# cy-rae/fast-slam

Measured on AMD Instinct MI355X. Metric: particle-updates/s, higher is better.
Workload: dtype f64

## Files before the change

fast-slam_amd/csrc/fs2_api.hip:

```cpp
#include <hip/hip_runtime.h>

#include <sched.h>
#include <unistd.h>

#include <algorithm>
#include <atomic>
#include <chrono>
#include <condition_variable>
#include <functional>
#include <cmath>
#include <cstdarg>
#include <cstdio>
#include <cstdlib>
#include <cstring>
#include <mutex>
#include <new>
#include <string>
#include <thread>
#include <tuple>
#include <vector>

#include "../../include/fs2.h"
#include "fs2_comm.hpp"
#include "fs2_frontend.hpp"
// ... 270 lines not shown
static void gm_free(GrowMem &g) {
    GmStep st{"free", g.mapped};
    size_t off = g.mapped;
    for (auto it = g.chunks.rbegin(); it != g.chunks.rend(); ++it) {
        off -= it->second;
        hipMemUnmap(g.base + off, it->second);
        gm_drop(g, it->second, it->first);
    }
    g.chunks.clear();
    if (g.base) hipMemAddressFree(g.base, g.reserved);
    g = GrowMem{};
}

struct Pool {
    const char *name;
    size_t item_bytes;
    int64_t id_limit;
    char *data = nullptr;
    int64_t n = 0;
    GrowMem vm;
    uint8_t *mark = nullptr;
    GrowMem mark_vm;
    uint32_t *freel = nullptr;
    GrowMem freel_vm;
    int64_t nfree = 0, cursor = 0;
    uint8_t epoch = 0;
    int64_t *bcnt = nullptr;
    int64_t bcnt_cap = 0;
    int64_t *nfree_dev = nullptr;

    int64_t room() const { return nfree - cursor; }
    int64_t live() const { return n - room(); }
    bool in_place() const { return vm.base && data == vm.base; }
    hipError_t next_epoch(hipStream_t s) {
        if (epoch == 255) {
            const hipError_t e = hipMemsetAsync(mark, 0, (size_t)n, s);
            if (e != hipSuccess) return e;
            epoch = 0;
        }
        epoch += 1;
        return hipSuccess;
    }
    bool mapped() const { return vm.base || mark_vm.base || freel_vm.base; }
    void release() {
        if (vm.base) gm_free(vm); else hipFree(data);
        if (mark_vm.base) gm_free(mark_vm); else hipFree(mark);
        if (freel_vm.base) gm_free(freel_vm); else hipFree(freel);
        hipFree(bcnt);
        hipFree(nfree_dev);
    }
};

}

struct MtCtx {
    fs2_mt_state in;
    double sigma = 0.0;
    int64_t N = 0, P = 0, A = 0, amb_cap = 0, pos0 = 0, have = 0, total = 0;
    int h0 = 0;
    fs2_mt_state *after = nullptr, *after_u0 = nullptr;
    double *u0_out = nullptr;
};

struct fs2_handle {
    fs2_config cfg{};
    int64_t n_global = 0, n = 0, first = 0;
    hipStream_t stream = nullptr;
    int cur = 0;
    double *x[2] = {}, *y[2] = {}, *yaw[2] = {}, *w[2] = {};
    int32_t *cnt[2] = {};
    Pool pages{"page", kPageBytes, (int64_t)kIdMask};
    Pool records{"record", kRecBytes, (int64_t)kRecIdLimit};
    Desc *pt[2] = {};
    uint32_t *bbox[2] = {};
    XDesc *rdesc = nullptr;
    XDesc *udesc = nullptr;
    size_t udesc_cap = 0;
    unsigned long long *xt_key = nullptr;
    uint32_t *xt_ref = nullptr, *xt_uidx = nullptr, *xt_cmask = nullptr, *xt_cbase = nullptr;
    uint32_t *xt_eslot = nullptr, *xt_ulist = nullptr;
    int64_t xt_cap = 0, xt_ecap = 0;
    SumFrame frame{-127.0f, 1.0f, 1.0f};
    float ext_seen = 0.0f;
    float *slb = nullptr;
    float *slb_pass = nullptr;
    uint32_t *ext_dev = nullptr;
    size_t rdesc_cap = 0;
    int rows = 0;
    uint32_t *sent_mask = nullptr;
    uint64_t collections = 0;
    int64_t u_recv = 0;
    int32_t *rank_d = nullptr, *rank_e = nullptr;
    int64_t *iblk = nullptr;
    int cap = 0, max_cap = kMaxSlots;
    double *wpart = nullptr, *part_sq = nullptr, *part_best_w = nullptr, *part_pose = nullptr;
    unsigned long long *cpart = nullptr;
    int64_t *part_best_i = nullptr;
    unsigned long long *part_slots = nullptr;
    int32_t *part_maxcnt = nullptr;
    double *cbuf = nullptr, *bsum = nullptr;
    DevStats *stats_dev = nullptr;
    char *post_host = nullptr, *post = nullptr;
    unsigned long long *post_flag = nullptr, *post_flag_dev = nullptr;
    unsigned long long post_seq = 0;
    PackPlan *plan = nullptr;
    DevStats *pub_stats = nullptr, *pub_stats_dev = nullptr;
    unsigned long long *pub_flag = nullptr, *pub_flag_dev = nullptr;
    unsigned long long pub_seq = 0;
    bool stats_clean = false;
    double *noise_dev = nullptr, *noise_pin = nullptr, *u0_dev = nullptr, *u0_pin = nullptr;
    struct MtWork {
        uint32_t *raw[2] = {};
        int64_t raw_cap[2] = {};
        int cur = 0;
        hipStream_t side = nullptr;
        hipEvent_t ev_words = nullptr, ev_pre = nullptr;
        bool pre_valid = false;
        uint32_t pre_key[2][624];
        int32_t pre_spos[2];
        int64_t pre_pos0[2];
        int64_t pre_total = 0;
        int32_t *boff = nullptr;
        int64_t boff_cap = 0;
        MtMeta *meta = nullptr, *meta_pin = nullptr;
        MtAmb *amb = nullptr, *amb_pin = nullptr;
        int64_t amb_cap = 0;
        uint32_t *words_pin = nullptr;
        int64_t *pidx = nullptr, *pidx_pin = nullptr;
        double *pval = nullptr, *pval_pin = nullptr;
        int64_t patch_cap = 0, pval_cap = 0;
        double *tab = nullptr;
        int64_t jJ = 0;
        int jG = 0;
        uint64_t *jpoly = nullptr;
        uint32_t *jwin = nullptr;
        bool tab_ready = false;
        bool armed = false;
        hipStream_t dstream = nullptr;
        hipEvent_t ev_in = nullptr, ev_noise = nullptr;
        bool deferred = false;
        MtCtx dc;
    } mt;
    int32_t *assoc_dev = nullptr;
    int64_t assoc_cap = 0;
    int32_t last_m = 0;
    uint64_t scan = 0;
    struct Pending {
        bool on = false;
        unsigned long long seq = 0;
        bool prof = false;
        int passes = 0;
        int32_t m = 0;
        uint64_t fixed_bytes = 0;
    } pending;
    struct TailCtx {
        int32_t M = 0;
        int passes = 0;
        uint64_t fixed_bytes = 0;
        bool prof = false;
        int evset = 0;
        int32_t want_collect = 0;
        bool has_u0 = false;
        int par = 0;
    };
    struct {
        bool on = false;
// ... 801 lines not shown
    for (int p = 0; p < G; ++p) {
        const bool so = p != keep && at(R, p, 0) > 0, ro = p != R && at(p, keep, 0) > 0;
        soff[p + 1] = soff[p] + (so ? arena_align((size_t)xfer_bytes(at(R, p, 0), at(R, p, 1), at(R, p, 2), at(R, p, 3))) : 0);
        roff[p + 1] = roff[p] + (ro ? arena_align((size_t)xfer_bytes(at(p, keep, 0), at(p, keep, 1), at(p, keep, 2),
                                                                      at(p, keep, 3))) : 0);
    }
    rc = ensure_arena(h, h->sarena, h->scap, soff[G]);
    if (!rc) rc = ensure_arena(h, h->rarena, h->rcap, roff[G]);
    if (rc) return rc;
    for (int p = 0; p < G; ++p) {
        rs.sbuf[p] = nullptr;
        T.ubase[p + 1] = T.ubase[p] + (p == keep ? 0 : at(R, p, 2));
        const int64_t K = at(R, p, 0), S = at(R, p, 1), U = at(R, p, 2), C = at(R, p, 3);
        if (log_xfer)
            std::fprintf(stderr,
                         "fs2 xfer scan %lld rank %d (shard %d -> %d) -> shard %d (rank %d)%s: %lld particles, "
                         "%lld rows, %lld pages, %lld covariances, %lld B\n",
                         (long long)h->scan, R, h->shard, keep, p, owner[p], p == keep ? " kept" : "", (long long)K,
                         (long long)S, (long long)U, (long long)C, (long long)(p == keep ? 0 : xfer_bytes(K, S, U, C)));
        if (p == keep || K == 0) continue;
        const size_t bytes = (size_t)xfer_bytes(K, S, U, C);
        rs.sbuf[p] = h->sarena + soff[p];
        sends.push_back({owner[p], rs.sbuf[p], bytes});
        nsend += K;
    }
    if (nsend > INT32_MAX) return set_err(&h->err, FS2_ERR_CAPACITY, "%lld particles to send", (long long)nsend);
    HIP_TRY(h, launch_pack_write(rs, s));
    rs.npeers = 0;
    int32_t kbase = 0;
    int64_t ubase = 0;
    for (int q = 0; q < G; ++q) {
        if (q == R) continue;
        const int64_t K = at(q, keep, 0), S = at(q, keep, 1), U = at(q, keep, 2), C = at(q, keep, 3);
        if (!K) continue;
        const size_t bytes = (size_t)xfer_bytes(K, S, U, C);
        char *rb = h->rarena + roff[q];
        recvs.push_back({q, rb, bytes});
        RecvPeer &pp = rs.peers[rs.npeers++];
        pp.hdr = reinterpret_cast<const PackHeader *>(rb);
        pp.idx = reinterpret_cast<const uint32_t *>(rb + xfer_idx_off(K));
        pp.pages = reinterpret_cast<const XferPage *>(rb + xfer_page_off(K, S));
        pp.covs = reinterpret_cast<const double2 *>(rb + xfer_cov_off(K, S, U));
        pp.K = (int32_t)K;
        pp.kbase = kbase;
        pp.U = U;
        pp.ubase = ubase;
        kbase += (int32_t)K;
        ubase += U;
    }
    rc = timed_exchange(h, sends, recvs, s);
    if (rc) return rc;
    h->n_recv = kbase;
    h->u_recv = ubase;
    if (h->profiling) {
        uint64_t np = 0, nr = 0, nu = 0, nb = 0;
        for (int p = 0; p < G; ++p) {
            if (p == keep) continue;
            np += at(R, p, 0);
            nr += at(R, p, 1);
            nu += at(R, p, 2);
            nb += at(R, p, 0) ? xfer_bytes(at(R, p, 0), at(R, p, 1), at(R, p, 2), at(R, p, 3)) : 0;
        }
        h->prof.migrations += np ? 1 : 0;
        h->prof.sent_particles += np;
        h->prof.sent_rows += nr;
        h->prof.sent_pages += nu;
        h->prof.sent_bytes += nb;
        h->prof.migrate_ms +=
            std::chrono::duration<double, std::milli>(std::chrono::steady_clock::now() - t_start).count();
    }
    rs.ao = shard_begin(h->n_global, G, keep);
    if (h->follow) {
        ResampleParams r2 = rs;
        r2.ranges_mode = 2;
        HIP_TRY(h, launch_resample_ranges(r2, s));
    }
    if (keep != h->shard) h->shard_moves += 1;
    h->shard = keep;
    h->first = rs.ao;
    for (int q = 0; q < G; ++q) h->rank_of[q] = (int8_t)owner[q];
    return FS2_OK;
}

static bool spatial_order(const double *lm, int L, std::vector<int32_t> &perm) {
    perm.resize(L);
    for (int j = 0; j < L; ++j) {
        perm[j] = j;
        if (!std::isfinite(lm[6 * j]) || !std::isfinite(lm[6 * j + 1])) return false;
    }
    struct Rec {
        static void go(const double *lm, int32_t *a, int n) {
            if (n <= kPageSlots) return;
            double x0 = INFINITY, x1 = -INFINITY, y0 = INFINITY, y1 = -INFINITY;
            for (int k = 0; k < n; ++k) {
                x0 = std::min(x0, lm[6 * a[k]]);
                x1 = std::max(x1, lm[6 * a[k]]);
                y0 = std::min(y0, lm[6 * a[k] + 1]);
                y1 = std::max(y1, lm[6 * a[k] + 1]);
            }
            const int ax = (x1 - x0 >= y1 - y0) ? 0 : 1;
            std::stable_sort(a, a + n, [&](int32_t u, int32_t v) { return lm[6 * u + ax] < lm[6 * v + ax]; });
            int h = ((n / 2 + kPageSlots - 1) / kPageSlots) * kPageSlots;
            if (h >= n) h = n - kPageSlots;
            go(lm, a, h);
            go(lm, a + h, n - h);
        }
    };
    Rec::go(lm, perm.data(), L);
    return true;
}

extern "C" {

int32_t fs2_abi_version(void) { return FS2_ABI_VERSION; }

#ifndef FS2_BUILD_ID
#define FS2_BUILD_ID "unknown"
#endif
const char *fs2_build_id(void) { return FS2_BUILD_ID; }

void fs2_config_default(fs2_config *c) {
    if (!c) return;
    std::memset(c, 0, sizeof *c);
    c->num_particles = 20;
    c->translation_noise = 0.0055;
    c->rotation_noise = 0.001;
    c->measurement_noise[0] = 0.001;
    c->measurement_noise[3] = 0.001;
    c->max_landmark_distance = 8.0;
    c->init_landmark_cov[0] = 0.1;
    c->init_landmark_cov[3] = 0.1;
    c->weight_floor = 1e-5;
    c->landmark_capacity = 64;
    c->max_landmark_capacity = 4096;
    c->device = 0;
    c->reduce_mode = FS2_REDUCE_AUTO;
    c->seed = 0x5EEDF5A2ull;
    c->record_assoc = 0;
    c->gate_filter = 1;
    c->rank = 0;
    c->world_size = 1;
}

const char *fs2_last_error(const fs2_handle *h) {
    if (h && !h->err.empty()) return h->err.c_str();
    return g_last_error.c_str();
}

static void free_handle(fs2_handle *h) {
    if (!h) return;
    int prev_dev = -1;
    if (hipGetDevice(&prev_dev) != hipSuccess) prev_dev = -1;
    if (prev_dev != h->cfg.device) (void)hipSetDevice(h->cfg.device);
    if (h->stream) hipStreamSynchronize(h->stream);
    if (h->mt.dstream) hipStreamSynchronize(h->mt.dstream);
    const bool vmm = h->pages.mapped() || h->records.mapped();
    if (vmm) hipDeviceSynchronize();
    if (h->refs_shared && h->tp && !h->tp->in_process()) {
        std::string e;
        if (h->tp->allgather(h->ep_dev, h->epochs_dev, 1, h->stream, &e) == FS2_OK) hipStreamSynchronize(h->stream);
        h->tp->unshare();
        if (h->tp->allgather(h->ep_dev, h->epochs_dev, 1, h->stream, &e) == FS2_OK) hipStreamSynchronize(h->stream);
    }
    for (int s = 0; s < 2; ++s) {
        hipFree(h->x[s]); hipFree(h->y[s]); hipFree(h->yaw[s]); hipFree(h->w[s]); hipFree(h->cnt[s]);
        hipFree(h->pt[s]);
        hipFree(h->bbox[s]);
    }
    hipFree(h->rdesc); hipFree(h->udesc);
    hipFree(h->xt_key); hipFree(h->xt_ref); hipFree(h->xt_uidx); hipFree(h->xt_cmask); hipFree(h->xt_cbase);
    hipFree(h->xt_eslot); hipFree(h->xt_ulist);
    hipFree(h->sent_mask);
    h->pages.release();
    h->records.release();
    if (vmm) hipDeviceSynchronize();
    hipFree(h->slb); hipFree(h->slb_pass); hipFree(h->ext_dev);
    hipFree(h->rank_d); hipFree(h->rank_e); hipFree(h->iblk);
    hipFree(h->mlo); hipFree(h->mhi); hipFree(h->out_src); hipFree(h->runs); hipFree(h->runs_n);
    hipFree(h->rec); hipFree(h->recs); hipFree(h->totals); hipFree(h->xrow); hipFree(h->xmat);
    hipFree(h->sarena);
    hipFree(h->rarena);
    hipFree(h->cand); hipFree(h->ncand);
    hipFree(h->uinfo); hipFree(h->uol); hipFree(h->seql); hipFree(h->udelta); hipFree(h->ugl);
    hipFree(h->bD); hipFree(h->bC); hipFree(h->bM); hipFree(h->bpd); hipFree(h->bpc);
    hipFree(h->uel); hipFree(h->bE); hipFree(h->bpe);
    hipFree(h->sout); hipFree(h->np_leaf); hipFree(h->part_w); hipFree(h->np_part); hipFree(h->np_tail);
    hipFree(h->urec); hipFree(h->sentry);
    hipFree(h->dch_send); hipFree(h->dch_recv); hipFree(h->recx); hipFree(h->recxs); hipFree(h->est_base);
    hipFree(h->uop); hipFree(h->np_tail_g);
    hipFree(h->peers_dev); hipFree(h->ep_dev); hipFree(h->epochs_dev);
    hipFree(h->part_pose);
    hipFree(h->gen_dev); hipFree(h->sets_dev); hipFree(h->go_dev);
// ... 1017 lines not shown
                                        (long long)capacity, (long long)need);
    if (m_out) *m_out = h->last_m;
    HIP_TRY(h, hipStreamSynchronize(h->stream));
    if (need) HIP_TRY(h, hipMemcpy(idx, h->assoc_dev, sizeof(int32_t) * need, hipMemcpyDeviceToHost));
    return FS2_OK;
}

static hipMemcpyKind kind_in(int32_t where) {
    return where == FS2_DEVICE ? hipMemcpyDeviceToDevice : hipMemcpyHostToDevice;
}
static hipMemcpyKind kind_out(int32_t where) {
    return where == FS2_DEVICE ? hipMemcpyDeviceToDevice : hipMemcpyDeviceToHost;
}

int fs2_set_state(fs2_handle *h, int64_t first, int64_t count, const double *x, const double *y,
                  const double *yaw, const double *w, const int32_t *cnt, const double *lm,
                  int32_t lm_cap, int32_t where) {
    if (!h) return set_err(nullptr, FS2_ERR_ARG, "null handle");
    if (h->pending.on) return set_err(&h->err, FS2_ERR_STATE, "a submitted scan is pending (fs2_iterate_wait first)");
    if (first < 0 || count < 0 || first + count > h->n)
        return set_err(&h->err, FS2_ERR_ARG, "range [%lld, %lld) outside %lld local particles",
                       (long long)first, (long long)(first + count), (long long)h->n);
    if ((cnt == nullptr) != (lm == nullptr) || (lm && lm_cap < 0))
        return set_err(&h->err, FS2_ERR_ARG, "cnt and lm must be given together");
    HIP_TRY(h, hipSetDevice(h->cfg.device));
    {
        const int rcm = mt_finish(h);
        h->mt.armed = false;
        if (rcm) return rcm;
    }
    hipStream_t s = h->stream;
    const int c = h->cur;
    HIP_TRY(h, hipStreamSynchronize(s));
    if (count == 0) return FS2_OK;
    const size_t b8 = sizeof(double) * count;
    if (x) HIP_TRY(h, copy_sync(h, h->x[c] + first, x, b8, kind_in(where)));
    if (y) HIP_TRY(h, copy_sync(h, h->y[c] + first, y, b8, kind_in(where)));
    if (yaw) HIP_TRY(h, copy_sync(h, h->yaw[c] + first, yaw, b8, kind_in(where)));
    if (w) HIP_TRY(h, copy_sync(h, h->w[c] + first, w, b8, kind_in(where)));
    if (cnt) {
        std::vector<int32_t> hc(count);
        HIP_TRY(h, hipMemcpy(hc.data(), cnt, sizeof(int32_t) * count,
                             where == FS2_DEVICE ? hipMemcpyDeviceToHost : hipMemcpyHostToHost));
        int32_t mx = 0;
        for (int32_t v : hc) {
            if (v < 0 || v > lm_cap) return set_err(&h->err, FS2_ERR_ARG, "count %d outside [0, %d]", v, lm_cap);
            mx = std::max(mx, v);
        }
        int rc = grow_rows(h, mx);
        if (rc) return rc;
        const int32_t rows_each = std::max(1, (mx + kPageSlots - 1) / kPageSlots);
        h->cnt_upper = std::max(h->cnt_upper, mx);
        {
            int64_t used = 0;
            for (int32_t v : hc) used += v;
            h->appends_since_rcollect += used;
            if ((int64_t)h->imported.size() != h->n) h->imported.assign((size_t)h->n, 0);
            bool replaced = h->scan > 0;
            for (int64_t k = first; k < first + count; ++k) {
                replaced |= h->imported[(size_t)k] != 0;
                h->imported[(size_t)k] = 1;
            }
            if (replaced) h->rcollect_exact = false;
        }
        const int64_t per = (int64_t)std::max(1, lm_cap) * 6 * 8;
        const int64_t chunk = std::max<int64_t>(1, (256ll << 20) / per);
        double *stage = nullptr;
        int32_t *cstage = nullptr, *perm_dev = nullptr;
        HIP_TRY(h, hipMemsetAsync(h->ext_dev, 0, sizeof(uint32_t), s));
        HIP_TRY(h, hipMalloc(&stage, (size_t)std::min(chunk, count) * per));
        HIP_TRY(h, hipMalloc(&cstage, sizeof(int32_t) * std::min(chunk, count)));
        HIP_TRY(h, hipMalloc(&perm_dev, sizeof(int32_t) * std::max(1, lm_cap)));
        std::vector<double> rep((size_t)std::max(1, lm_cap) * 6);
        std::vector<int32_t> perm;
        int rc2 = FS2_OK;
        for (int64_t o = 0; o < count && rc2 == FS2_OK; o += chunk) {
            const int64_t k = std::min(chunk, count - o);
            hipError_t e = copy_sync(h, stage, lm + o * lm_cap * 6, (size_t)k * per, kind_in(where));
            if (e == hipSuccess) e = hipMemcpy(cstage, hc.data() + o, sizeof(int32_t) * k, hipMemcpyHostToDevice);
            int32_t perm_len = -1;
            if (e == hipSuccess && h->cfg.gate_filter && hc[o] > kPageSlots) {
                e = hipMemcpy(rep.data(), lm + o * lm_cap * 6, sizeof(double) * 6 * (size_t)hc[o],
                              where == FS2_DEVICE ? hipMemcpyDeviceToHost : hipMemcpyHostToHost);
                if (e == hipSuccess && spatial_order(rep.data(), hc[o], perm)) {
                    perm_len = hc[o];
                    e = hipMemcpy(perm_dev, perm.data(), sizeof(int32_t) * perm_len, hipMemcpyHostToDevice);
                }
            }
            PageAlloc pa{};
            rc2 = reserve_recs(h, k * std::max(1, lm_cap), &pa);
            if (rc2) break;
            rc2 = reserve_pages(h, k * rows_each, &pa);
            if (rc2) break;
            if (e == hipSuccess)
                e = launch_import(stage, cstage, first + o, k, lm_cap, h->map(), pa, rows_each, h->cnt[c], h->ext_dev,
                                  perm_len > 0 ? perm_dev : nullptr, perm_len, s);
            if (e == hipSuccess) e = hipStreamSynchronize(s);
            if (e != hipSuccess) rc2 = set_err(&h->err, FS2_ERR_HIP, "state import failed: %s", hipGetErrorString(e));
        }
        hipFree(stage);
        hipFree(cstage);
        hipFree(perm_dev);
        if (rc2) return rc2;
        uint32_t eb = 0;
        HIP_TRY(h, hipMemcpy(&eb, h->ext_dev, sizeof eb, hipMemcpyDeviceToHost));
        float ext = 0.0f;
        std::memcpy(&ext, &eb, sizeof ext);
        h->ext_seen = std::max(h->ext_seen, ext);
#ifdef FS2_AB_POW2_CELL
        float cell = 1.0f / 64.0f;
        while (127.0f * cell < 1.25f * h->ext_seen && cell < 65536.0f) cell *= 2.0f;
#else
        float cell = (float)std::max(1.0, std::ceil(1.25 * (double)h->ext_seen / 127.0 * 64.0)) / 64.0f;
        if (!(cell < 65536.0f)) cell = 65536.0f;
#endif
        if (cell != h->frame.cell) h->frame = SumFrame{-127.0f * cell, cell, 1.0f / cell};
        HIP_TRY(h, launch_bbox_build(h->map(), h->cnt[c], s));
    }
    HIP_TRY(h, hipStreamSynchronize(s));
    return FS2_OK;
}

int fs2_update_known_landmarks(fs2_handle *h, double eps, double min_fraction, double *centres, int64_t cap,
                               int64_t *n_clusters) {
    if (!h || !n_clusters || (cap > 0 && !centres) || !(eps > 0.0))
        return set_err(h ? &h->err : nullptr, FS2_ERR_ARG, "fs2_update_known_landmarks: bad arguments");
    if (h->pending.on) return set_err(&h->err, FS2_ERR_STATE, "a submitted scan is pending (fs2_iterate_wait first)");
    if (h->cfg.world_size > 1)
        return set_err(&h->err, FS2_ERR_STATE, "update_known_landmarks needs every particle on one rank");
    HIP_TRY(h, hipSetDevice(h->cfg.device));
    hipStream_t s = h->stream;
    HIP_TRY(h, hipStreamSynchronize(s));
    double2 *pts = nullptr;
    int64_t np = 0;
    HIP_TRY(h, gather_map_points(h->map(), h->cnt[h->cur], h->n, &pts, &np, s));
    const double avg = (double)np / (double)h->n_global;
    const double ms = avg * min_fraction;
    if (!(ms >= 1.0)) {
        (void)hipFree(pts);
        *n_clusters = -1;
        return FS2_OK;
    }
    int32_t status = 0;
    int64_t K = 0;
    double *dcent = nullptr;
    hipError_t e = hipMalloc(&dcent, sizeof(double) * 2 * std::max<int64_t>(cap, 1));
    if (e == hipSuccess)
        e = cluster_points(pts, np, eps, (int64_t)ms, dcent, cap, &K, nullptr, &status, s);
    if (e == hipSuccess && K <= cap && K > 0)
        e = hipMemcpy(centres, dcent, sizeof(double) * 2 * K, hipMemcpyDeviceToHost);
    (void)hipFree(pts);
    (void)hipFree(dcent);
    if (e != hipSuccess) return set_err(&h->err, FS2_ERR_HIP, "update_known_landmarks: %s", hipGetErrorString(e));
    if (status == 1) return set_err(&h->err, FS2_ERR_ARG, "Input contains NaN or infinity");
    if (status == 2) return set_err(&h->err, FS2_ERR_ARG, "landmark coordinates span too many eps-cells");
    *n_clusters = K;
    if (K > cap) return set_err(&h->err, FS2_ERR_ARG, "%lld clusters, centre buffer holds %lld", (long long)K,
                                (long long)cap);
    return FS2_OK;
}

int fs2_get_state(fs2_handle *h, int64_t first, int64_t count, double *x, double *y, double *yaw,
                  double *w, int32_t *cnt, double *lm, int32_t lm_cap, int32_t where) {
    if (!h) return set_err(nullptr, FS2_ERR_ARG, "null handle");
    if (h->pending.on) return set_err(&h->err, FS2_ERR_STATE, "a submitted scan is pending (fs2_iterate_wait first)");
    if (first < 0 || count < 0 || first + count > h->n)
        return set_err(&h->err, FS2_ERR_ARG, "range outside local particles");
    HIP_TRY(h, hipSetDevice(h->cfg.device));
// ... 995 lines not shown
        HIP_TRY(h, hipMemcpyAsync(mt.raw[nx], mt.raw[mt.cur] + kMtN * kb1, 4 * (size_t)keep,
                                  hipMemcpyDeviceToDevice, mt.side));
        {
            int64_t made = 0;
            const int rcf = mt_fill(h, mt.raw[nx], keep, want, mt.side, &made);
            if (rcf) return rcf;
            want = made;
        }
        HIP_TRY(h, hipEventRecord(mt.ev_pre, mt.side));
        std::memcpy(mt.pre_key[0], after->key, sizeof mt.pre_key[0]);
        std::memcpy(mt.pre_key[1], after_u0->key, sizeof mt.pre_key[1]);
        mt.pre_spos[0] = after->pos;
        mt.pre_spos[1] = after_u0->pos;
        mt.pre_pos0[0] = after->pos;
        mt.pre_pos0[1] = kMtN * (kb2 - kb1) + after_u0->pos;
        mt.pre_total = want;
        mt.pre_valid = true;
    }
    const uint32_t wu[2] = {meta.w_u0[0], meta.w_u0[1]};
    const double hi = 1.0 / (double)h->n_global;
    const double u0 = 0.0 + (hi - 0.0) * mt_double(mt_temper(wu[0]), mt_temper(wu[1]));
    *h->u0_pin = u0;
    HIP_TRY(h, hipMemcpyAsync(h->u0_dev, h->u0_pin, 8, hipMemcpyHostToDevice, s));
    if (c.u0_out) *c.u0_out = u0;
    return FS2_OK;
}

static int mt_finish(fs2_handle *h) {
    auto &mt = h->mt;
    if (!mt.deferred) return FS2_OK;
    mt.deferred = false;
    const int rc = mt_end(h, mt.dc, mt.dstream);
    HIP_TRY(h, hipEventRecord(mt.ev_noise, mt.dstream));
    HIP_TRY(h, hipStreamWaitEvent(h->stream, mt.ev_noise, 0));
    if (rc) return rc;
    mt.armed = true;
    return FS2_OK;
}

int fs2_mt_draw(fs2_handle *h, const fs2_mt_state *in, double sigma, fs2_mt_state *after,
                fs2_mt_state *after_u0, double *u0_out) {
    if (!h) return set_err(nullptr, FS2_ERR_ARG, "null handle");
    HIP_TRY(h, hipSetDevice(h->cfg.device));
    int rc = mt_finish(h);
    if (rc) return rc;
    h->mt.armed = false;
    MtCtx c;
    rc = mt_begin(h, in, sigma, after, after_u0, u0_out, h->stream, c);
    if (rc) return rc;
    rc = mt_end(h, c, h->stream);
    if (rc) return rc;
    h->mt.armed = true;
    return FS2_OK;
}

int fs2_mt_draw_deferred(fs2_handle *h, const fs2_mt_state *in, double sigma, fs2_mt_state *after,
                         fs2_mt_state *after_u0, double *u0_out) {
    if (!h) return set_err(nullptr, FS2_ERR_ARG, "null handle");
    HIP_TRY(h, hipSetDevice(h->cfg.device));
    auto &mt = h->mt;
    int rc = mt_finish(h);
    if (rc) return rc;
    mt.armed = false;
    if (!mt.dstream) {
        HIP_TRY(h, hipStreamCreateWithFlags(&mt.dstream, hipStreamNonBlocking));
        HIP_TRY(h, hipEventCreateWithFlags(&mt.ev_in, hipEventDisableTiming));
        HIP_TRY(h, hipEventCreateWithFlags(&mt.ev_noise, hipEventDisableTiming));
    }
    HIP_TRY(h, hipEventRecord(mt.ev_in, h->stream));
    HIP_TRY(h, hipStreamWaitEvent(mt.dstream, mt.ev_in, 0));
    MtCtx &c = mt.dc;
    rc = mt_begin(h, in, sigma, after, after_u0, u0_out, mt.dstream, c);
    if (rc) return rc;
    mt.deferred = true;
    return FS2_OK;
}

int fs2_debug_mt_jump(const uint32_t key[624], uint64_t J, uint32_t out[624]) {
    if (!key || !out) return set_err(nullptr, FS2_ERR_ARG, "fs2_debug_mt_jump: null argument");
    if (!mt_jump_host(key, J, out)) return set_err(nullptr, FS2_ERR_STATE, "MT19937 characteristic polynomial not found");
    return FS2_OK;
}

int64_t fs2_release_cached_memory(void) { return (int64_t)g_chunks.release(); }

int fs2_debug_vm_fail_after_relocate(int32_t on) {
    g_vm_fail_after_relocate.store(on ? 1 : 0);
    return FS2_OK;
}

int fs2_debug_refuse_peer_maps(fs2_handle *h) {
    if (!h) return set_err(nullptr, FS2_ERR_ARG, "null handle");
    if (h->refs_shared || h->refs_off)
        return set_err(&h->err, FS2_ERR_STATE, "fs2_debug_refuse_peer_maps: the pools are mapped already");
    h->refuse_maps = true;
    return FS2_OK;
}

int fs2_debug_noise(fs2_handle *h, double *out) {
    if (!h || !out) return set_err(h ? &h->err : nullptr, FS2_ERR_ARG, "fs2_debug_noise: null argument");
    HIP_TRY(h, hipSetDevice(h->cfg.device));
    {
        const int rcm = mt_finish(h);
        if (rcm) return rcm;
    }
    HIP_TRY(h, hipMemcpyAsync(h->noise_pin, h->noise_dev, sizeof(double) * h->n, hipMemcpyDeviceToHost, h->stream));
    HIP_TRY(h, hipStreamSynchronize(h->stream));
    std::memcpy(out, h->noise_pin, sizeof(double) * h->n);
    return FS2_OK;
}

int64_t fs2_debug_check_guards(fs2_handle *h, char *first_bad, int64_t len) {
    if (!h) return set_err(nullptr, FS2_ERR_ARG, "fs2_debug_check_guards: null handle");
    if (first_bad && len > 0) first_bad[0] = 0;
    HIP_TRY(h, hipSetDevice(h->cfg.device));
    HIP_TRY(h, hipStreamSynchronize(h->stream));
    std::vector<unsigned char> buf(kGuardBytes);
    int64_t bad = 0;
    for (const auto &g : h->guards) {
        HIP_TRY(h, hipMemcpy(buf.data(), g.at, kGuardBytes, hipMemcpyDeviceToHost));
        int64_t k = 0;
        for (unsigned char c : buf) k += c != (unsigned char)kGuardByte;
        if (k && first_bad && len > 0 && !first_bad[0]) std::snprintf(first_bad, (size_t)len, "%s", g.name);
        bad += k;
    }
    return bad;
}

int fs2_debug_weights(fs2_handle *h, int32_t other, double *out) {
    if (!h || !out) return set_err(h ? &h->err : nullptr, FS2_ERR_ARG, "fs2_debug_weights: null argument");
    HIP_TRY(h, hipSetDevice(h->cfg.device));
    HIP_TRY(h, hipStreamSynchronize(h->stream));
    HIP_TRY(h, hipMemcpy(out, h->w[other ? 1 - h->cur : h->cur], sizeof(double) * (size_t)h->n, hipMemcpyDeviceToHost));
    return FS2_OK;
}

int64_t fs2_debug_out_src(fs2_handle *h, int32_t *out, int64_t capacity) {
    if (!h || !out || capacity < h->n)
        return set_err(h ? &h->err : nullptr, FS2_ERR_ARG, "fs2_debug_out_src: null argument or capacity < n");
    HIP_TRY(h, hipSetDevice(h->cfg.device));
    HIP_TRY(h, hipStreamSynchronize(h->stream));
    HIP_TRY(h, hipMemcpy(out, h->out_src, sizeof(int32_t) * (size_t)h->n, hipMemcpyDeviceToHost));
    return h->n;
}

int fs2_debug_mt_log(int32_t device, const double *x, int64_t n, double *out, int32_t *amb, int32_t on_host) {
    if (n < 0 || (n > 0 && (!x || !out || !amb))) return set_err(nullptr, FS2_ERR_ARG, "fs2_debug_mt_log: bad arguments");
    if (on_host) {
        double thi[kMtLogTab], tlo[kMtLogTab];
        for (int k = 0; k < kMtLogTab; ++k) {
            const DD l = mt_log_tab_entry(k);
            thi[k] = l.hi;
            tlo[k] = l.lo;
        }
        for (int64_t k = 0; k < n; ++k) {
            bool a = false;
            out[k] = mt_log(x[k], thi, tlo, &a);
            amb[k] = a ? 1 : 0;
        }
        return FS2_OK;
    }
    if (n == 0) return FS2_OK;
    std::lock_guard<std::mutex> lk(g_scratch_mu);
    const size_t b8 = al16((size_t)n * 8);
    Scratch *sc = nullptr;
    int rc = scratch_get(device, 2 * b8 + al16((size_t)n * 4), &sc);
// ... 762 lines not shown
```

fast-slam_amd/fast_slam_2/_native.py:

```python
from __future__ import annotations

import ctypes as C
import os
import sys

import numpy as np

_PKG = os.path.dirname(os.path.abspath(__file__))
LIB_PATH = os.environ.get("FS2_LIB", os.path.join(os.path.dirname(_PKG), "lib", "libfs2.so"))

FS2_OK = 0
FS2_ERR_ARG = -1
FS2_ERR_HIP = -2
FS2_ERR_OOM = -3
FS2_ERR_LINALG = -4
FS2_ERR_STATE = -5
FS2_ERR_COMM = -6
FS2_ERR_CAPACITY = -7

FS2_REDUCE_AUTO = 0
FS2_REDUCE_SEQUENTIAL = 1
FS2_REDUCE_PARALLEL = 2
FS2_REDUCE_EXACT = 3
FS2_HOST = 0
# ... 146 lines not shown
    def __init__(self, code, msg):
        super().__init__(f"libfs2 error {code}: {msg}")
        self.code = code


_dp = C.POINTER(C.c_double)
_ip = C.POINTER(C.c_int32)
_vp = C.c_void_p
_H = C.c_void_p

SIGNATURES = [
    ("fs2_abi_version", C.c_int32, []),
    ("fs2_build_id", C.c_char_p, []),
    ("fs2_config_default", None, [C.POINTER(fs2_config)]),
    ("fs2_create", C.c_int, [C.POINTER(fs2_config), C.POINTER(_H)]),
    ("fs2_destroy", None, [_H]),
    ("fs2_last_error", C.c_char_p, [_H]),
    ("fs2_iterate", C.c_int, [_H, C.c_double, C.c_double, _vp, _vp, C.c_int32, _vp, _vp, _dp,
                              C.POINTER(fs2_iter_stats)]),
    ("fs2_iterate_submit", C.c_int, [_H, C.c_double, C.c_double, _vp, _vp, C.c_int32, _vp, _vp]),
    ("fs2_iterate_wait", C.c_int, [_H, _dp, C.POINTER(fs2_iter_stats)]),
    ("fs2_mt_draw", C.c_int, [_H, C.POINTER(fs2_mt_state), C.c_double, C.POINTER(fs2_mt_state),
                              C.POINTER(fs2_mt_state), _dp]),
    ("fs2_mt_draw_deferred", C.c_int, [_H, C.POINTER(fs2_mt_state), C.c_double, C.POINTER(fs2_mt_state),
                                       C.POINTER(fs2_mt_state), _dp]),
    ("fs2_get_state", C.c_int, [_H, C.c_int64, C.c_int64, _vp, _vp, _vp, _vp, _vp, _vp, C.c_int32,
                                C.c_int32]),
    ("fs2_set_state", C.c_int, [_H, C.c_int64, C.c_int64, _vp, _vp, _vp, _vp, _vp, _vp, C.c_int32,
                                C.c_int32]),
    ("fs2_snapshot_save", C.c_int, [_H, _vp, C.c_int64, C.POINTER(C.c_int64)]),
    ("fs2_snapshot_save_select", C.c_int, [_H, _vp, C.c_int64, _vp, C.c_int64, C.POINTER(C.c_int64)]),
    ("fs2_snapshot_load", C.c_int, [_H, _vp, C.c_int64]),
    ("fs2_snapshot_check", C.c_int, [_vp, C.c_int64, C.POINTER(fs2_snapshot_info)]),
    ("fs2_get_assoc", C.c_int, [_H, _ip, C.c_int64, _ip]),
    ("fs2_shard_info", C.c_int, [_H, C.POINTER(C.c_int64), C.POINTER(C.c_int64),
                                 C.POINTER(C.c_int32)]),
    ("fs2_synchronize", C.c_int, [_H]),
    ("fs2_set_profiling", C.c_int, [_H, C.c_int32]),
    ("fs2_get_profile", C.c_int, [_H, C.POINTER(fs2_profile)]),
    ("fs2_icp", C.c_int, [C.c_int32, _dp, C.c_int32, _dp, C.c_int32, C.c_int32, C.c_double, _dp,
                          _dp, _ip]),
    ("fs2_icp_submit", C.c_int, [C.c_int32, _dp, C.c_int32, _dp, C.c_int32, C.c_int32, C.c_double,
                                 C.POINTER(C.c_int64)]),
    ("fs2_icp_wait", C.c_int, [C.c_int32, C.c_int64, _dp, _dp, _ip]),
    ("fs2_icp_batched", C.c_int, [C.c_int32, C.c_int32, C.c_int32, _vp, _vp, C.c_int32,
                                  C.c_double, _vp, _vp, _vp, C.c_int32]),
    ("fs2_best_fit_transform", C.c_int, [C.c_int32, _dp, _dp, C.c_int32, _dp, _dp]),
    ("fs2_line_filter", C.c_int, [C.c_int32, _dp, C.c_int32, _dp, C.c_int32, _dp]),
    ("fs2_gaussian_taps", C.c_int32, [C.c_double, C.c_double, _dp, C.c_int32]),
    ("fs2_associate", C.c_int, [C.c_int32, _dp, _dp, C.c_int32, C.c_double, _ip]),
    ("fs2_mahalanobis", C.c_int, [C.c_int32, _dp, _dp, _dp, C.c_int32, _dp]),
    ("fs2_cluster_points", C.c_int, [C.c_int32, _vp, C.c_int64, C.c_double, C.c_int64, _vp, C.c_int64,
                                     C.POINTER(C.c_int64), _vp, C.c_int32]),
    ("fs2_update_known_landmarks", C.c_int, [_H, C.c_double, C.c_double, _dp, C.c_int64,
                                             C.POINTER(C.c_int64)]),
    ("fs2_frontend", C.c_int, [C.c_int32, C.c_int32, _vp, _vp, C.c_int32, _dp, C.c_int32, C.c_int32,
                               C.POINTER(fs2_frontend_out)]),
    ("fs2_repr_doubles", C.c_int, [C.c_int32, _vp, C.c_int64, _vp, _vp, C.c_int32]),
    ("fs2_poses_json", C.c_int, [C.c_int32, _vp, _vp, _vp, C.c_int64, C.c_int32, _vp, C.c_int64,
                                 C.POINTER(C.c_int64), C.c_int32]),
    ("fs2_particles_json", C.c_int, [_H, C.c_int64, C.c_int64, C.c_int32, _vp, C.c_int64,
                                     C.POINTER(C.c_int64)]),
    ("fs2_debug_json_times", C.c_int, [C.c_int32, _vp]),
    ("fs2_pose_moments", C.c_int, [_H, C.c_int32, _vp, _vp, _vp, _vp]),
    ("fs2_pose_density", C.c_int, [_H, C.c_int32, C.c_double, C.c_double, C.c_double, C.c_int32, C.c_int32, _vp,
                                   C.POINTER(C.c_int32), C.POINTER(C.c_uint64)]),
    ("fs2_density_scale", C.c_int, [C.c_double, C.c_int64, C.POINTER(C.c_int32)]),
    ("fs2_debug_posterior_times", C.c_int, [C.c_int32, _vp]),
    ("fs2_map_summary", C.c_int, [_H, _vp, _vp]),
    ("fs2_map_density", C.c_int, [_H, C.c_int32, C.c_double, C.c_double, C.c_double, C.c_int32, C.c_int32, _vp,
                                  C.POINTER(C.c_int32), C.POINTER(C.c_uint64)]),
    ("fs2_debug_map_times", C.c_int, [C.c_int32, _vp]),
    ("fs2_debug_philox", C.c_int, [C.c_int32, C.c_int64, _vp, _vp, _vp]),
    ("fs2_debug_normals", C.c_int, [C.c_int32, C.c_uint64, C.c_uint64, C.c_uint64, C.c_int64, _vp]),
    ("fs2_debug_mt_log", C.c_int, [C.c_int32, _vp, C.c_int64, _vp, _vp, C.c_int32]),
    ("fs2_debug_refuse_peer_maps", C.c_int, [_H]),
    ("fs2_debug_vm_fail_after_relocate", C.c_int, [C.c_int32]),
    ("fs2_release_cached_memory", C.c_int64, []),
    ("fs2_debug_noise", C.c_int, [_H, _vp]),
    ("fs2_debug_out_src", C.c_int64, [_H, _vp, C.c_int64]),
    ("fs2_debug_weights", C.c_int, [_H, C.c_int32, _vp]),
    ("fs2_debug_check_guards", C.c_int64, [_H, C.c_char_p, C.c_int64]),
    ("fs2_debug_mt_jump", C.c_int, [_vp, C.c_uint64, _vp]),
    ("fs2_comm_unique_id", C.c_int, [C.POINTER(C.c_uint8)]),
    ("fs2_plan_ranges", C.c_int, [_vp, C.c_int64, C.c_int64, C.c_int64, C.c_double, C.c_double, _vp, _vp]),
    ("fs2_plan_sends", C.c_int, [_vp, _vp, _vp, C.c_int64, C.c_int64, C.c_int32, C.c_int32, _vp, _vp, _vp]),
]

_lib = None


HIP_RUNTIME = None


def _wheel_hip_version(torch_dir):
    try:
        for line in open(os.path.join(torch_dir, "version.py")):
            if line.startswith("hip"):
                v = line.split("=", 1)[1].strip().strip("'\"")
                return None if v in ("None", "") else v
    except OSError:
        pass
    return None


def _system_hip_version():
    try:
        return open(os.path.join(os.environ.get("ROCM_PATH", "/opt/rocm"), ".info", "version")).read().strip()
    except OSError:
        return None


def _share_torch_hip_runtime():
    global HIP_RUNTIME
    want = os.environ.get("FS2_HIP_RUNTIME", "").strip().lower()
    sysv = _system_hip_version()
    HIP_RUNTIME = ("system", None, sysv)
    if want == "system":
        return
    torch_dirs = []
    if "torch" in sys.modules and getattr(sys.modules["torch"], "__file__", None):
        torch_dirs = [os.path.dirname(sys.modules["torch"].__file__)]
    else:
        try:
            import importlib.util
            spec = importlib.util.find_spec("torch")
        except Exception:
            spec = None
        if spec is not None and spec.submodule_search_locations:
            torch_dirs = list(spec.submodule_search_locations)
    for d in torch_dirs:
        p = os.path.join(d, "lib", "libamdhip64.so")
        if not os.path.exists(p):
            continue
        try:
            C.CDLL(p, mode=C.RTLD_GLOBAL)
        except OSError:
            return
        wv = _wheel_hip_version(d)
        HIP_RUNTIME = ("torch-wheel", p, wv)
        if wv and sysv and wv.split(".")[:2] != sysv.split(".")[:2]:
            import warnings
            warnings.warn(f"libfs2 runs on PyTorch's HIP runtime {wv} ({p}), not the system ROCm {sysv} it "
                          f"was compiled against (one runtime per process; FS2_HIP_RUNTIME=system opts out)",
                          RuntimeWarning, stacklevel=3)
        break
    if os.environ.get("FS2_VERBOSE"):
        print(f"[fs2] HIP runtime: {HIP_RUNTIME}", file=sys.stderr)


def load():
    global _lib
    if _lib is not None:
        return _lib
    if not os.path.exists(LIB_PATH):
        raise ImportError(f"libfs2.so not found at {LIB_PATH}; build it with "
                          f"`python fast-slam_amd/build.py` (there is no CPU fallback)")
    _share_torch_hip_runtime()
    lib = C.CDLL(LIB_PATH)
    for name, res, args in SIGNATURES:
        fn = getattr(lib, name)
        fn.restype = res
        fn.argtypes = args
    if lib.fs2_abi_version() != 2:
        raise ImportError(f"libfs2 ABI {lib.fs2_abi_version()} != 2")
    _lib = lib
# ... 45 lines not shown
```

include/fs2.h:

```cpp
#ifndef FS2_H
#define FS2_H

#include <stdint.h>

#ifdef __cplusplus
extern "C" {
#endif

#define FS2_ABI_VERSION 2

enum {
    FS2_OK = 0,
    FS2_ERR_ARG = -1,
    FS2_ERR_HIP = -2,
    FS2_ERR_OOM = -3,
    FS2_ERR_LINALG = -4,
    FS2_ERR_STATE = -5,
    FS2_ERR_COMM = -6,
    FS2_ERR_CAPACITY = -7
};

enum {
    FS2_REDUCE_AUTO = 0,
    FS2_REDUCE_SEQUENTIAL = 1,
// ... 155 lines not shown
int fs2_snapshot_load(fs2_handle *h, const void *buf, int64_t size);
int fs2_snapshot_check(const void *buf, int64_t size, fs2_snapshot_info *info);

int fs2_get_assoc(fs2_handle *h, int32_t *idx, int64_t capacity, int32_t *m_out);

int fs2_shard_info(const fs2_handle *h, int64_t *n_local, int64_t *first_global,
                   int32_t *capacity);

int fs2_synchronize(fs2_handle *h);

int fs2_set_profiling(fs2_handle *h, int32_t enable);
int fs2_get_profile(const fs2_handle *h, fs2_profile *out);


int fs2_icp(int32_t device, const double *src, int32_t n_src, const double *tgt,
            int32_t n_tgt, int32_t max_iterations, double threshold, double R[4],
            double t[2], int32_t *iterations);

#define FS2_ICP_SLOTS 4
int fs2_icp_submit(int32_t device, const double *src, int32_t n_src, const double *tgt,
                   int32_t n_tgt, int32_t max_iterations, double threshold, int64_t *ticket);
int fs2_icp_wait(int32_t device, int64_t ticket, double R[4], double t[2], int32_t *iterations);

int fs2_icp_batched(int32_t device, int32_t B, int32_t P, const double *src,
                    const double *tgt, int32_t max_iterations, double threshold, double *R,
                    double *t, int32_t *iterations, int32_t where);

int fs2_best_fit_transform(int32_t device, const double *src, const double *tgt, int32_t n,
                           double R[4], double t[2]);

int fs2_line_filter(int32_t device, const double *points, int32_t n, const double *taps,
                    int32_t radius, double *out);

int32_t fs2_gaussian_taps(double sigma, double truncate, double *taps, int32_t max_taps);

int fs2_associate(int32_t device, const double observed[2], const double *lm, int32_t L,
                  double gate, int32_t *index);

int fs2_mahalanobis(int32_t device, const double *a, const double *b, const double *cov,
                    int32_t K, double *out);


int fs2_repr_doubles(int32_t device, const double *v, int64_t n, char *out, uint8_t *len,
                     int32_t on_host);

int fs2_poses_json(int32_t device, const double *x, const double *y, const double *yaw,
                   int64_t n, int32_t depth, char *buf, int64_t capacity, int64_t *size,
                   int32_t where);

int fs2_particles_json(fs2_handle *h, int64_t first, int64_t count, int32_t depth, char *buf,
                       int64_t capacity, int64_t *size);

int fs2_debug_json_times(int32_t enable, double ms[4]);


int fs2_pose_moments(fs2_handle *h, int32_t weighted, double mean[3], double cov[9], double sums[4],
                     double bbox[4]);

int fs2_pose_density(fs2_handle *h, int32_t weighted, double x0, double y0, double cell,
                     int32_t nx, int32_t ny, uint64_t *grid, int32_t *scale_exp, uint64_t *outside);

int fs2_debug_posterior_times(int32_t enable, double ms[2]);


int fs2_map_summary(fs2_handle *h, double bbox[4], int64_t counts[4]);

int fs2_map_density(fs2_handle *h, int32_t weighted, double x0, double y0, double cell,
                    int32_t nx, int32_t ny, uint64_t *grid, int32_t *scale_exp, uint64_t *outside);

int fs2_debug_map_times(int32_t enable, double ms[3]);

int fs2_debug_philox(int32_t device, int64_t n, const uint32_t *ctr, const uint32_t *key, uint32_t *out);
int fs2_debug_normals(int32_t device, uint64_t seed, uint64_t stream, uint64_t first, int64_t n,
                      double *out);
int fs2_debug_mt_log(int32_t device, const double *x, int64_t n, double *out, int32_t *amb,
                     int32_t on_host);
int fs2_debug_refuse_peer_maps(fs2_handle *h);
int fs2_debug_vm_fail_after_relocate(int32_t on);
int fs2_debug_noise(fs2_handle *h, double *out);
int64_t fs2_debug_out_src(fs2_handle *h, int32_t *out, int64_t capacity);
int fs2_debug_weights(fs2_handle *h, int32_t other, double *out);
int64_t fs2_debug_check_guards(fs2_handle *h, char *first_bad, int64_t len);
int fs2_debug_mt_jump(const uint32_t key[624], uint64_t J, uint32_t out[624]);


int fs2_cluster_points(int32_t device, const double *points, int64_t n, double eps,
                       int64_t min_samples, double *centres, int64_t cap, int64_t *n_clusters,
                       int32_t *labels, int32_t where);

int fs2_update_known_landmarks(fs2_handle *h, double eps, double min_fraction, double *centres,
                               int64_t cap, int64_t *n_clusters);


typedef struct fs2_frontend_out {
    int32_t cap;
    float *lines;
    double *intersections;
    double *clusters;
    double *corners;
    double *measurements;
    int32_t *counts;
} fs2_frontend_out;

int fs2_frontend(int32_t device, int32_t B, const int64_t *offsets, const double *points,
                 int32_t where, const double *taps, int32_t radius, int32_t legacy,
                 fs2_frontend_out *out);

int fs2_comm_unique_id(uint8_t out[128]);

int fs2_plan_ranges(const double *c, int64_t n, int64_t first_global, int64_t N, double offset, double u0,
                    int32_t *mlo, int32_t *mhi);
int fs2_plan_sends(const int32_t *mlo, const int32_t *mhi, const int32_t *cnt, int64_t n, int64_t N,
                   int32_t world, int32_t rank, int64_t *run, int64_t *K, int64_t *S);

int fs2_density_scale(double wmax, int64_t n, int32_t *e);

#ifdef __cplusplus
}
#endif

#endif
```

Baseline: 457.7 million.

## Choose landmark page layout by gate-aware bounding-box cost among several split orders

Measured after the change: 379.7 million. -17.0%, worse.

```diff
diff --git a/fast-slam_amd/csrc/fs2_api.hip b/fast-slam_amd/csrc/fs2_api.hip
--- a/fast-slam_amd/csrc/fs2_api.hip
+++ b/fast-slam_amd/csrc/fs2_api.hip
@@ -376,6 +376,7 @@
     int64_t xt_cap = 0, xt_ecap = 0;
     SumFrame frame{-127.0f, 1.0f, 1.0f};
     float ext_seen = 0.0f;
+    std::vector<int32_t> layout_perm;
     float *slb = nullptr;
     float *slb_pass = nullptr;
     uint32_t *ext_dev = nullptr;
@@ -1343,32 +1344,163 @@
     return FS2_OK;
 }
 
-static bool spatial_order(const double *lm, int L, std::vector<int32_t> &perm) {
+namespace layout {
+
+constexpr int kBisect = 1, kLookAhead = 3, kOrders = 3;
+[[maybe_unused]] constexpr double kKeepFactor = 1.1;
+
+static inline double px(const double *lm, int32_t j, int ax) { return lm[6 * j + ax]; }
+
+static bool finite_xy(const double *lm, int L) {
+    for (int j = 0; j < L; ++j)
+        if (!std::isfinite(lm[6 * j]) || !std::isfinite(lm[6 * j + 1])) return false;
+    return true;
+}
+
+static inline int pages_of(int n) { return (n + kPageSlots - 1) / kPageSlots; }
+
+static double order_cost(const double *lm, const int32_t *perm, int L, double e) {
+    double C = 0.0;
+    for (int p = 0; p < L; p += kPageSlots) {
+        double x0 = INFINITY, x1 = -INFINITY, y0 = INFINITY, y1 = -INFINITY;
+        for (int k = p; k < std::min(L, p + kPageSlots); ++k) {
+            x0 = std::min(x0, px(lm, perm[k], 0));
+            x1 = std::max(x1, px(lm, perm[k], 0));
+            y0 = std::min(y0, px(lm, perm[k], 1));
+            y1 = std::max(y1, px(lm, perm[k], 1));
+        }
+        C += (x1 - x0 + e) * (y1 - y0 + e);
+    }
+    return C;
+}
+
+static void bisect(const double *lm, int32_t *a, int n) {
+    if (n <= kPageSlots) return;
+    double x0 = INFINITY, x1 = -INFINITY, y0 = INFINITY, y1 = -INFINITY;
+    for (int k = 0; k < n; ++k) {
+        x0 = std::min(x0, lm[6 * a[k]]);
+        x1 = std::max(x1, lm[6 * a[k]]);
+        y0 = std::min(y0, lm[6 * a[k] + 1]);
+        y1 = std::max(y1, lm[6 * a[k] + 1]);
+    }
+    const int ax = (x1 - x0 >= y1 - y0) ? 0 : 1;
+    std::stable_sort(a, a + n, [&](int32_t u, int32_t v) { return lm[6 * u + ax] < lm[6 * v + ax]; });
+    int h = ((n / 2 + kPageSlots - 1) / kPageSlots) * kPageSlots;
+    if (h >= n) h = n - kPageSlots;
+    bisect(lm, a, h);
+    bisect(lm, a + h, n - h);
+}
+
+static double child_score(double w, double h, int k, double e, bool ahead) {
+    if (!ahead) return (w + e) * (h + e);
+    double best = INFINITY;
+    for (int a = 1; a <= k; ++a) {
+        const int b = (k + a - 1) / a;
+        best = std::min(best, (double)k * (w / a + e) * (h / b + e));
+        if (b == 1) break;
+    }
+    return best;
+}
+
+struct Scratch {
+    std::vector<int32_t> s[2];
+    std::vector<double> lo, hi;
+};
+
+static void split(const double *lm, int32_t *a, int n, double e, bool ahead, Scratch &sc) {
+    if (n <= kPageSlots) return;
+    double best = INFINITY;
+    int best_h = std::min(pages_of(n / 2) * kPageSlots, (pages_of(n) - 1) * kPageSlots), best_ax = 0;
+    for (int ax = 0; ax < 2; ++ax) {
+        std::vector<int32_t> &s = sc.s[ax];
+        s.assign(a, a + n);
+        std::stable_sort(s.begin(), s.end(), [&](int32_t u, int32_t v) { return px(lm, u, ax) < px(lm, v, ax); });
+        sc.lo.resize(n + 1);
+        sc.hi.resize(n + 1);
+        sc.lo[n] = INFINITY;
+        sc.hi[n] = -INFINITY;
+        for (int k = n - 1; k >= 0; --k) {
+            sc.lo[k] = std::min(sc.lo[k + 1], px(lm, s[k], 1 - ax));
+            sc.hi[k] = std::max(sc.hi[k + 1], px(lm, s[k], 1 - ax));
+        }
+        double plo = INFINITY, phi = -INFINITY;
+        for (int k = 0; k < n; ++k) {
+            if (k && k % kPageSlots == 0) {
+                const double wl = px(lm, s[k - 1], ax) - px(lm, s[0], ax), hl = phi - plo;
+                const double wr = px(lm, s[n - 1], ax) - px(lm, s[k], ax), hr = sc.hi[k] - sc.lo[k];
+                const double c = child_score(wl, hl, k / kPageSlots, e, ahead) +
+                                 child_score(wr, hr, pages_of(n - k), e, ahead);
+                const bool closer = std::abs(2 * k - n) < std::abs(2 * best_h - n);
+                if (c < best || (c == best && closer)) {
+                    best = c;
+                    best_h = k;
+                    best_ax = ax;
+                }
+            }
+            plo = std::min(plo, px(lm, s[k], 1 - ax));
+            phi = std::max(phi, px(lm, s[k], 1 - ax));
+        }
+    }
+    std::copy(sc.s[best_ax].begin(), sc.s[best_ax].end(), a);
+    split(lm, a, best_h, e, ahead, sc);
+    split(lm, a + best_h, n - best_h, e, ahead, sc);
+}
+
+static double build(const double *lm, int L, double e, int which, int32_t *perm) {
+    for (int j = 0; j < L; ++j) perm[j] = j;
+    if (which == kBisect) {
+        bisect(lm, perm, L);
+    } else {
+        Scratch sc;
+        split(lm, perm, L, e, which == kLookAhead, sc);
+    }
+    return order_cost(lm, perm, L, e);
+}
+
+static int choose(const double *lm, int L, double e, std::vector<int32_t> &perm, double *cost) {
     perm.resize(L);
+    int best = kBisect;
+    double cb = build(lm, L, e, kBisect, perm.data());
+#ifndef FS2_AB_BISECT_LAYOUT
+    std::vector<int32_t> t(L);
+    for (int w = kBisect + 1; w <= kOrders; ++w) {
+        const double c = build(lm, L, e, w, t.data());
+        if (c < cb) {
+            cb = c;
+            best = w;
+            perm.swap(t);
+        }
+    }
+#endif
+    if (cost) *cost = cb;
+    return best;
+}
+
+static double slack(const double *lm, int L, double gate2f) {
+    double smin = INFINITY, ext = 0.0;
     for (int j = 0; j < L; ++j) {
-        perm[j] = j;
-        if (!std::isfinite(lm[6 * j]) || !std::isfinite(lm[6 * j + 1])) return false;
-    }
-    struct Rec {
-        static void go(const double *lm, int32_t *a, int n) {
-            if (n <= kPageSlots) return;
-            double x0 = INFINITY, x1 = -INFINITY, y0 = INFINITY, y1 = -INFINITY;
-            for (int k = 0; k < n; ++k) {
-                x0 = std::min(x0, lm[6 * a[k]]);
-                x1 = std::max(x1, lm[6 * a[k]]);
-                y0 = std::min(y0, lm[6 * a[k] + 1]);
-                y1 = std::max(y1, lm[6 * a[k] + 1]);
-            }
-            const int ax = (x1 - x0 >= y1 - y0) ? 0 : 1;
-            std::stable_sort(a, a + n, [&](int32_t u, int32_t v) { return lm[6 * u + ax] < lm[6 * v + ax]; });
-            int h = ((n / 2 + kPageSlots - 1) / kPageSlots) * kPageSlots;
-            if (h >= n) h = n - kPageSlots;
-            go(lm, a, h);
-            go(lm, a + h, n - h);
-        }
-    };
-    Rec::go(lm, perm.data(), L);
-    return true;
+        const double *q = lm + 6 * j;
+        ext = std::max(ext, std::max(std::fabs((double)(float)q[0]), std::fabs((double)(float)q[1])));
+        const double det = q[2] * q[5] - q[3] * q[4];
+        if (!(std::isfinite(det) && det != 0.0)) continue;
+        const double a = q[5] / det, c = q[2] / det, b = -0.5 * (q[3] + q[4]) / det;
+        const double half = 0.5 * (a + c), dd = 0.5 * (a - c);
+        const double lmax = half + std::sqrt(dd * dd + b * b);
+        const double lmin = (a * c - b * b) / lmax;
+        if (!(lmin > 0.0 && lmax < 1e300 && lmax <= 1e8 * lmin)) continue;
+        float s = (float)(lmin * (1.0 - 1e-6));
+        uint32_t u;
+        std::memcpy(&u, &s, sizeof u);
+        u &= ~0xfffu;
+        std::memcpy(&s, &u, sizeof s);
+        if (s > 0.0f) smin = std::min(smin, (double)s);
+    }
+    double cell = std::max(1.0, std::ceil(1.25 * ext / 127.0 * 64.0)) / 64.0;
+    if (!(cell < 65536.0)) cell = 65536.0;
+    const double R = std::sqrt(gate2f / smin);
+    return (std::isfinite(R) ? 2.0 * R : 0.0) + cell;
+}
+
 }
 
 extern "C" {
@@ -2552,8 +2684,19 @@
             if (e == hipSuccess && h->cfg.gate_filter && hc[o] > kPageSlots) {
                 e = hipMemcpy(rep.data(), lm + o * lm_cap * 6, sizeof(double) * 6 * (size_t)hc[o],
                               where == FS2_DEVICE ? hipMemcpyDeviceToHost : hipMemcpyHostToHost);
-                if (e == hipSuccess && spatial_order(rep.data(), hc[o], perm)) {
+                if (e == hipSuccess && layout::finite_xy(rep.data(), hc[o])) {
                     perm_len = hc[o];
+                    const double gate2f = std::isinf(h->gate2) ? INFINITY : h->gate2 / (1.0 - 0x1p-18);
+                    const double le = layout::slack(rep.data(), perm_len, gate2f);
+                    double fresh = 0.0;
+                    layout::choose(rep.data(), perm_len, le, perm, &fresh);
+#ifndef FS2_AB_BISECT_LAYOUT
+                    if ((int32_t)h->layout_perm.size() == perm_len &&
+                        layout::order_cost(rep.data(), h->layout_perm.data(), perm_len, le) <= layout::kKeepFactor * fresh)
+                        perm = h->layout_perm;
+                    else
+                        h->layout_perm = perm;
+#endif
                     e = hipMemcpy(perm_dev, perm.data(), sizeof(int32_t) * perm_len, hipMemcpyHostToDevice);
                 }
             }
@@ -3715,6 +3858,26 @@
     return FS2_OK;
 }
 
+int fs2_debug_layout(const double *lm, int32_t L, double e, int32_t which, int32_t *perm_out, double *cost_out) {
+    if (!lm || !perm_out || L < 1 || L > kMaxSlots || which < 0 || which > layout::kOrders || !(e >= 0.0) ||
+        !std::isfinite(e))
+        return set_err(nullptr, FS2_ERR_ARG, "fs2_debug_layout: bad arguments");
+    int got = 0;
+    double cost = NAN;
+    if (!layout::finite_xy(lm, L)) {
+        for (int32_t j = 0; j < L; ++j) perm_out[j] = j;
+    } else if (which == 0) {
+        std::vector<int32_t> perm;
+        got = layout::choose(lm, L, e, perm, &cost);
+        std::copy(perm.begin(), perm.end(), perm_out);
+    } else {
+        cost = layout::build(lm, L, e, which, perm_out);
+        got = which;
+    }
+    if (cost_out) *cost_out = cost;
+    return got;
+}
+
 int64_t fs2_release_cached_memory(void) { return (int64_t)g_chunks.release(); }
 
 int fs2_debug_vm_fail_after_relocate(int32_t on) {
diff --git a/fast-slam_amd/fast_slam_2/_native.py b/fast-slam_amd/fast_slam_2/_native.py
--- a/fast-slam_amd/fast_slam_2/_native.py
+++ b/fast-slam_amd/fast_slam_2/_native.py
@@ -252,6 +252,7 @@
     ("fs2_debug_weights", C.c_int, [_H, C.c_int32, _vp]),
     ("fs2_debug_check_guards", C.c_int64, [_H, C.c_char_p, C.c_int64]),
     ("fs2_debug_mt_jump", C.c_int, [_vp, C.c_uint64, _vp]),
+    ("fs2_debug_layout", C.c_int, [_vp, C.c_int32, C.c_double, C.c_int32, _vp, _vp]),
     ("fs2_comm_unique_id", C.c_int, [C.POINTER(C.c_uint8)]),
     ("fs2_plan_ranges", C.c_int, [_vp, C.c_int64, C.c_int64, C.c_int64, C.c_double, C.c_double, _vp, _vp]),
     ("fs2_plan_sends", C.c_int, [_vp, _vp, _vp, C.c_int64, C.c_int64, C.c_int32, C.c_int32, _vp, _vp, _vp]),
diff --git a/include/fs2.h b/include/fs2.h
--- a/include/fs2.h
+++ b/include/fs2.h
@@ -261,6 +261,7 @@
 int fs2_debug_weights(fs2_handle *h, int32_t other, double *out);
 int64_t fs2_debug_check_guards(fs2_handle *h, char *first_bad, int64_t len);
 int fs2_debug_mt_jump(const uint32_t key[624], uint64_t J, uint32_t out[624]);
+int fs2_debug_layout(const double *lm, int32_t L, double e, int32_t which, int32_t *perm_out, double *cost_out);
 
 
 int fs2_cluster_points(int32_t device, const double *points, int64_t n, double eps,
```
